# amansanghvi/Thesis

Measured on AMD Instinct MI355X. Metric: particle-updates/sec (particles x scans/s) @1081 beams, higher is better.
Workload: dtype int8 map cells (lattice log-odds), f64 poses/weights; 1 GPU; BASELINE configs[2]: room16 synthetic, 4096 particles/GPU, 1081 beams, 0.05 m grid, K=30 samples, both matcher stages, resample every step; particles_per_gpu=4096, beams=1081, parallelism=particles sharded x1

## Files before the change

thesis_amd/csrc/kernels_match.hip:

```cpp
#include <limits.h>
#include <string.h>

#include <hip/hip_ext.h>

#include "rbpf_internal.h"
#include "rbpf_device.h"

namespace rbpf {

#ifdef RBPF_STAMPS
#define MSTAMP(k) do { if (tid == 0) { long long t_ = clock64(); st_acc[k] += t_ - st_prev; st_prev = t_; } } while (0)
#else
#define MSTAMP(k) do { } while (0)
#endif

static const int MBLOCK = 512;
static const int M_COARSE = 4;
static const int M_FINE_T = 4;
static const int M_FINE_R = 4;

struct MatchArgs {
    int mode;
    int single;
    const double* ref_xy; int n_ref;
// ... 7 lines not shown
    double max_range;
    const float* sel_x; const float* sel_y; int n_sel;
    int n_coarse_rot;
    int cap_sel;
    int sc_cap;
    int p0;
    double cell_off;
    int ndt;
    int ndt_nc;
    int ndt_max_iter;
    const int32_t* dup_of;
    uint32_t* ndt_occ;
    double* ndt_aux;
};

struct __attribute__((packed, aligned(4))) MaskPair { uint32_t lo, hi; };
struct __attribute__((packed, aligned(4))) MaskTriple { uint32_t w0, w1, w2; };

struct MatchLds {
    uint32_t* occ;
    uint32_t* dil;
    uint32_t* crs;
    float* fx4; float* fy4;
    float* cx8; float* cy8;
    int* sc;
};

__host__ __device__ inline int match_crs_words(int N) { return ((N / M_COARSE) + 15) / 16; }
static const int CRS_PAD = 7;
__host__ __device__ inline int match_crs_stride(int N) { return N / M_COARSE + 2 * CRS_PAD; }
// ... 18 lines not shown
    if (nsc > (size_t)n_coarse && (size_t)n_coarse >= fine) nsc = (size_t)n_coarse;
    return base + nsc * 4;
}
int match_sc_capacity(int N, int B, size_t lds) { return (int)((lds - match_lds_base(N, B)) / 4); }

template <int N>
__device__ __forceinline__ double dpp_row_shl_f64(double x) {
    const unsigned long long b = __builtin_bit_cast(unsigned long long, x);
    const int lo = __builtin_amdgcn_update_dpp(0, (int)(uint32_t)b, 0x100 + N, 0xF, 0xF, true);
    const int hi = __builtin_amdgcn_update_dpp(0, (int)(uint32_t)(b >> 32), 0x100 + N, 0xF, 0xF, true);
    return __builtin_bit_cast(double, ((unsigned long long)(uint32_t)hi << 32) | (uint32_t)lo);
}
__device__ __forceinline__ double wave_sum_lane0_f64(double x) {
    x += __shfl_down(x, 32, 64); x += __shfl_down(x, 16, 64);
    x += dpp_row_shl_f64<8>(x); x += dpp_row_shl_f64<4>(x); x += dpp_row_shl_f64<2>(x); x += dpp_row_shl_f64<1>(x);
    return x;
}

__device__ __forceinline__ int field_hit(const MatchLds& s, int N, int u, int w) {
    if ((unsigned)u >= (unsigned)N || (unsigned)w >= (unsigned)N) return 0;
    int idx = u * (N >> 5) + (w >> 5);
    uint32_t m = 1u << (w & 31);
    return ((s.occ[idx] & m) ? 1 : 0) + ((s.dil[idx] & m) ? 1 : 0);
}
__device__ inline void match_frame_from(const MatchArgs& a, const double* pose5, double* g, double* rng, int* org) {
    double gx, gy, gth, rx, ry;
    if (a.single) {
        gx = a.guess[0]; gy = a.guess[1]; gth = a.guess[2]; rx = a.range[0]; ry = a.range[1];
    } else {
        gx = pose5[0]; gy = pose5[1]; gth = pose5[2];
// ... 23 lines not shown
    if (dup != p) { if (tid == 0) atomicAdd(&v.stats[ST_MATCH_SHARED], 1ull); return; }
    MatchLds s;
    s.occ = reinterpret_cast<uint32_t*>(smem);
    s.dil = s.occ + (size_t)N * W;
    s.crs = s.dil + (size_t)N * W;
    const int cap4 = ((a.cap_sel + 3) / 4 + 7) & ~3, cap8 = ((a.cap_sel + 7) / 8 + 7) & ~3;
    s.fx4 = reinterpret_cast<float*>(s.crs + match_crs_total(N)); s.fy4 = s.fx4 + cap4;
    s.cx8 = s.fy4 + cap4; s.cy8 = s.cx8 + cap8;
    s.sc = reinterpret_cast<int*>(s.cy8 + cap8);
    __shared__ double s_g[3], s_rng[2];
    __shared__ int s_org[2], s_nb, s_best;
    __shared__ unsigned long long s_bestc;
    __shared__ unsigned s_def[32], s_slowg;
    __shared__ double s_mom[10], s_wmom[MBLOCK / 64][10];
    __shared__ int s_tab[49];

#ifdef RBPF_STAMPS
    long long st_acc[8] = {0, 0, 0, 0, 0, 0, 0, 0}, st_prev = clock64();
#endif
    if (tid == 0) {
        match_frame_from(a, pre, s_g, s_rng, s_org);
        s_nb = 0; s_best = INT_MIN; s_bestc = 0ull; s_slowg = 0;
        for (int i = 0; i < 10; ++i) s_mom[i] = 0.0;
    }
    if (!a.single) {
        const int32_t* tab = v.tile_tab + (size_t)pre_slot * v.L * v.L;
        for (int i = tid; i < v.L * v.L; i += MBLOCK) s_tab[i] = tab[i];
    }
    if (a.mode != 0) for (int i = tid; i < N * W; i += MBLOCK) s.occ[i] = 0;
    if (tid < 32) s_def[tid] = 0;
    __syncthreads();
    const int ox = s_org[0], oy = s_org[1];

    MSTAMP(0);
    if (a.mode == 0) {
        int16_t* colmap = reinterpret_cast<int16_t*>(s.sc);
        uint32_t* rowbase = s.dil;
        for (int i = tid; i < N * a.ds; i += MBLOCK) {
            const int gyi = oy * a.ds + i, gxi = ox * a.ds + i;
            int16_t e = -1;
            if (lut_valid_g(v, gyi)) {
                const uint32_t ey = lut_at(v, gyi);
                e = (int16_t)((lut_lat(ey) << 12) | lut_cidx(ey));
                const int dev_ = lut_cidx(ey) - (gyi - (lut_lat(ey) - v.R) * v.dim + v.dim / 2);
                if (dev_ == -1) atomicOr(&s_def[(i >> 5) & 31], 1u << (i & 31));
                else if (dev_ != 0) atomicOr(&s_slowg, 1u << ((i >> 5) & 31));
                const int g0 = gyi - (i & 31);
                if ((i & 31) && !(lut_valid_g(v, g0) && lut_lat(lut_at(v, g0)) == lut_lat(ey))) atomicOr(&s_slowg, 1u << ((i >> 5) & 31));
            } else atomicOr(&s_slowg, 1u << ((i >> 5) & 31));
            colmap[i] = e;
            uint32_t rb = 0xFFFFFFFFu;
            if (lut_valid_g(v, gxi)) { const uint32_t ex = lut_at(v, gxi); rb = ((uint32_t)lut_lat(ex) << 24) | (uint32_t)lut_cidx(ex); }
            rowbase[i] = rb;
        }
        __syncthreads();
        MSTAMP(6);
        if (a.ds == 2 && 2 * W <= 32 && !v.match_stage_slow) {
            for (int q = tid; q < N * W; q += MBLOCK) {
                const int u = q / W, wv = q % W;
                const int e0 = colmap[wv * 64], e1 = colmap[wv * 64 + 32];
                const bool fast2 = !((s_slowg >> (2 * wv)) & 3u) && e0 >= 0 && e1 >= 0 && (e0 >> 12) == (e1 >> 12);
                uint32_t bits = 0;
                if (fast2) {
                    const int lat = e0 >> 12;
                    const int c0 = (oy * 2 + wv * 64) - (lat - v.R) * v.dim + v.dim / 2;
                    const int cy = max(c0 - 1, 0), wi = cy >> 5, sft = c0 - (wi << 5);
                    const unsigned long long d64 = ((unsigned long long)s_def[2 * wv + 1] << 32) | s_def[2 * wv];
                    unsigned long long acc = 0;
                    for (int du = 0; du < 2; ++du) {
                        const uint32_t rb = rowbase[u * 2 + du];
                        if (rb == 0xFFFFFFFFu) continue;
                        const int t = s_tab[(rb >> 24) * v.L + lat];
                        if (t < 0) continue;
                        const uint32_t* row = v.occ + ((size_t)t * v.dim + (rb & 0xFFFFFFu)) * v.ow;
// ... 20 lines not shown
                        if (rb == 0xFFFFFFFFu) continue;
                        for (int b = 0; b < 64; ++b) {
                            const int e = colmap[wv * 64 + b];
                            if (e < 0) continue;
                            const int t = s_tab[(rb >> 24) * v.L + (e >> 12)];
                            if (t < 0) continue;
                            const int cyb = e & 0xFFF;
                            const uint32_t wd = v.occ[((size_t)t * v.dim + (rb & 0xFFFFFFu)) * v.ow + (cyb >> 5)];
                            if ((wd >> (cyb & 31)) & 1u) bits |= 1u << (b >> 1);
                        }
                    }
                }
                s.occ[u * W + wv] = bits;
            }
        } else {
        const int SW = 4;
        const int GT = (W + 3) / 4, NRB = N / 16;
        const unsigned slowg = (a.ds != 1 || W > 32 || v.match_stage_slow) ? 0xFFFFFFFFu : s_slowg;
        const int wave = tid >> 6, ln = tid & 63;
        for (int g = 0; g < GT; ++g) {
            const int wv = g * 4 + (ln >> 4);
            const bool wv_ok = wv < W, fastw = wv_ok && !((slowg >> wv) & 1u);
            int lat = 0, wi = 0, sft = 0; uint32_t d = 0;
            if (fastw) {
                lat = colmap[wv * 32] >> 12;
                const int c0 = (oy + wv * 32) - (lat - v.R) * v.dim + v.dim / 2;
                wi = max(c0 - 1, 0) >> 5;
                sft = c0 - (wi << 5);
                d = s_def[wv];
            }
            for (int rb0 = wave; rb0 < NRB; rb0 += SW * (MBLOCK / 64)) {
                MaskPair mp[SW];
#pragma unroll
                for (int k = 0; k < SW; ++k) {
                    const int rbk = rb0 + k * (MBLOCK / 64);
                    mp[k].lo = 0; mp[k].hi = 0;
                    if (rbk >= NRB || !fastw) continue;
                    const uint32_t rb = rowbase[rbk * 16 + (ln & 15)];
                    if (rb == 0xFFFFFFFFu) continue;
                    const int t = s_tab[(rb >> 24) * v.L + lat];
                    if (t < 0) continue;
                    mp[k] = *reinterpret_cast<const MaskPair*>(v.occ + ((size_t)t * v.dim + (rb & 0xFFFFFFu)) * v.ow + wi);
                }
#pragma unroll
                for (int k = 0; k < SW; ++k) {
                    const int rbk = rb0 + k * (MBLOCK / 64), u = rbk * 16 + (ln & 15);
                    if (rbk >= NRB || !wv_ok) continue;
                    uint32_t bits;
                    if (fastw) {
                        const unsigned long long w01 = ((unsigned long long)mp[k].hi << 32) | mp[k].lo;
                        bits = sft < 32 ? (uint32_t)(w01 >> sft) : mp[k].hi;
                        if (d) {
                            const int s1 = sft - 1;
                            const uint32_t below = s1 < 0 ? bits << 1 : (uint32_t)(w01 >> s1);
                            bits = (bits & ~d) | (below & d);
                        }
                    } else {
                        bits = 0;
                        for (int du = 0; du < a.ds; ++du) {
                            const uint32_t rb = rowbase[u * a.ds + du];
                            if (rb == 0xFFFFFFFFu) continue;
                            for (int b = 0; b < 32 * a.ds; ++b) {
                                const int e = colmap[wv * 32 * a.ds + b];
                                if (e < 0) continue;
                                const int t = s_tab[(rb >> 24) * v.L + (e >> 12)];
                                if (t < 0) continue;
                                const int cy = e & 0xFFF;
                                const uint32_t wd = v.occ[((size_t)t * v.dim + (rb & 0xFFFFFFu)) * v.ow + (cy >> 5)];
                                if ((wd >> (cy & 31)) & 1u) bits |= 1u << (b / a.ds);
                            }
                        }
                    }
                    s.occ[u * W + wv] = bits;
                }
            }
        }
        }
        __syncthreads();
    } else {
        const int RP = 4;
        for (int i0 = tid; i0 < a.n_ref; i0 += RP * MBLOCK) {
          double2 pt[RP];
#pragma unroll
          for (int k = 0; k < RP; ++k) { const int i = i0 + k * MBLOCK; pt[k] = i < a.n_ref ? reinterpret_cast<const double2*>(a.ref_xy)[i] : make_double2(0.0, 0.0); }
#pragma unroll
          for (int k = 0; k < RP; ++k) {
            if (i0 + k * MBLOCK >= a.n_ref) continue;
            double rx = pt[k].x, ry = pt[k].y;
            double dx = rx - s_g[0], dy = ry - s_g[1];
            if (!(sqrt(dx * dx + dy * dy) < a.max_range)) continue;
            int u = (int)floor(rx / a.mcs + a.cell_off) - ox, w = (int)floor(ry / a.mcs + a.cell_off) - oy;
            if ((unsigned)u < (unsigned)N && (unsigned)w < (unsigned)N) atomicOr(&s.occ[u * W + (w >> 5)], 1u << (w & 31));
          }
        }
    }
    {
        const float inv = (float)(1.0 / a.mcs);
        const float FAR = -1.0e6f;
        for (int i = tid; i < cap4; i += MBLOCK) { const int b = 4 * i; const bool ok = b < a.n_sel; s.fx4[i] = ok ? a.sel_x[b] * inv : FAR; s.fy4[i] = ok ? a.sel_y[b] * inv : FAR; }
        for (int i = tid; i < cap8; i += MBLOCK) { const int b = 8 * i; const bool ok = b < a.n_sel; s.cx8[i] = ok ? a.sel_x[b] * inv : FAR; s.cy8[i] = ok ? a.sel_y[b] * inv : FAR; }
        if (tid == 0) s_nb = a.n_sel;
    }
    __syncthreads();
    if (a.ndt_occ) {
        uint32_t* dst = a.ndt_occ + (size_t)p * N * W;
        for (int i = tid; i < N * W; i += MBLOCK) dst[i] = s.occ[i];
    }
    MSTAMP(1);
    {
        const int nchunk = max(1, MBLOCK / W), rows_per = (N + nchunk - 1) / nchunk;
        const int wv = tid % W, chunk = tid / W;
        const bool row16 = W == 16;
        auto hdil = [&](int u) -> uint32_t {
            const bool inr = u >= 0 && u < N;
            const uint32_t c = inr ? s.occ[u * W + wv] : 0u;
            uint32_t lb, rb;
            if (row16) {
                lb = (uint32_t)__builtin_amdgcn_update_dpp(0, (int)(c >> 31), 0x111, 0xF, 0xF, true);
                rb = (uint32_t)__builtin_amdgcn_update_dpp(0, (int)(c << 31), 0x101, 0xF, 0xF, true);
            } else {
                lb = (inr && wv > 0) ? s.occ[u * W + wv - 1] >> 31 : 0u;
                rb = (inr && wv + 1 < W) ? s.occ[u * W + wv + 1] << 31 : 0u;
            }
            return c | (c << 1) | (c >> 1) | lb | rb;
        };
        if (chunk < nchunk) {
            const int u0 = chunk * rows_per, u1 = min(N, u0 + rows_per);
            uint32_t up = hdil(u0 - 1), mid = hdil(u0);
            for (int u = u0; u < u1; ++u) {
                const uint32_t dn = hdil(u + 1);
                s.dil[u * W + wv] = up | mid | dn;
                up = mid; mid = dn;
            }
        }
    }
    __syncthreads();
    for (int q = tid; q < (N / M_COARSE) * match_crs_words(N); q += MBLOCK) {
        const int cu = q / match_crs_words(N), h = q % match_crs_words(N);
        uint32_t out = 0;
#pragma unroll
        for (int k = 0; k < 4; ++k) {
            const int wv = 2 * h + k;
// ... 267 lines not shown
            for (int k = 0; k < 9; ++k) o[3 + k] = NAN;
            o[12] = 0.0;
        } else {
            const double sw = s_mom[0];
            double mu[3] = {s_mom[1] / sw, s_mom[2] / sw, s_mom[3] / sw};
            double c[3][3];
            c[0][0] = s_mom[4] / sw - mu[0] * mu[0]; c[0][1] = s_mom[5] / sw - mu[0] * mu[1]; c[0][2] = s_mom[6] / sw - mu[0] * mu[2];
            c[1][1] = s_mom[7] / sw - mu[1] * mu[1]; c[1][2] = s_mom[8] / sw - mu[1] * mu[2]; c[2][2] = s_mom[9] / sw - mu[2] * mu[2];
            c[1][0] = c[0][1]; c[2][0] = c[0][2]; c[2][1] = c[1][2];
            const double fl_t = (a.mcs * a.mcs) / 16.0, fl_r = (a.d0 * a.d0) / 16.0;
            c[0][0] = fmax(c[0][0], 0.0) + fl_t; c[1][1] = fmax(c[1][1], 0.0) + fl_t; c[2][2] = fmax(c[2][2], 0.0) + fl_r;
            for (int i = 0; i < 3; ++i) for (int j = 0; j < 3; ++j) o[3 + 3 * i + j] = c[i][j];
            o[12] = 0.5 * (double)full_score;
        }
        if (a.ndt_aux) {
            double* x = a.ndt_aux + (size_t)p * 5;
            x[0] = bdx / a.mcs; x[1] = bdy / a.mcs; x[2] = bth; x[3] = (double)full_score; x[4] = ok ? 1.0 : 0.0;
        }
    }
}

struct NdtCell { double mx, my, b00, b01, b11; };
__device__ inline bool ndt_cell_stats(int n, int sx, int sy, int sxx, int sxy, int syy, NdtCell& c) {
    if (n < 3) return false;
    const double nn = (double)n, mx = (double)sx / nn, my = (double)sy / nn;
    const double ca = ((double)sxx - (double)sx * mx) / (nn - 1.0);
    const double cb = ((double)sxy - (double)sx * my) / (nn - 1.0);
    const double cc = ((double)syy - (double)sy * my) / (nn - 1.0);
    const double half_tr = 0.5 * (ca + cc), disc = sqrt(0.25 * (ca - cc) * (ca - cc) + cb * cb);
    const double l1 = half_tr + disc, l2 = half_tr - disc;
    double k = 0.0;
    if (l2 < 1e-3 * l1) { k = (1e-3 * l1 - l2) / (l1 - l2); if (!(fabs(k) <= 1.79e308)) k = 0.0; }
// ... 111 lines not shown
__global__ __launch_bounds__(NBLOCK, 4) void ndt_kernel(DevView v, MatchArgs a) {
    extern __shared__ __align__(16) unsigned char smem[];
    const int N = a.N, W = N >> 5, tid = threadIdx.x, p = a.p0 + blockIdx.x;
    uint32_t* occ = reinterpret_cast<uint32_t*>(smem);
    const float* __restrict__ bx = a.sel_x;
    const float* __restrict__ by = a.sel_y;
    const float inv = (float)(1.0 / a.mcs);
    __shared__ double s_g[3], s_rng[2], s_trial[6], s_w[NBLOCK / 64][10];
    __shared__ int s_org[2], s_go;
    __shared__ float s_lut[5][16];
    __shared__ unsigned s_ok;
#ifdef RBPF_STAMPS
    long long st_acc[8] = {0, 0, 0, 0, 0, 0, 0, 0}, st_prev = clock64();
#endif
    if (a.dup_of && a.dup_of[p] != p) return;
    const double* aux = a.ndt_aux + (size_t)p * 5;
    if (aux[4] == 0.0 || a.n_sel <= 0) return;
    if (tid == 0) { match_frame(v, a, p, s_g, s_rng, s_org); s_ok = 0; }
    const int WPD = W + 2;
    {
        const uint32_t* src = a.ndt_occ + (size_t)p * N * W;
        int u = tid / W, wv = tid % W;
        const int du = NBLOCK / W, dw = NBLOCK % W;
        const int SL = 16;
        for (int i0 = tid; i0 < N * W; i0 += SL * NBLOCK) {
            uint32_t val[SL]; int dst[SL];
#pragma unroll
            for (int k = 0; k < SL; ++k) {
                const int i = i0 + k * NBLOCK;
                val[k] = i < N * W ? src[i] : 0u;
                dst[k] = (u + 1) * WPD + wv + 1;
                u += du; wv += dw;
                if (wv >= W) { wv -= W; ++u; }
            }
#pragma unroll
            for (int k = 0; k < SL; ++k)
                if (i0 + k * NBLOCK < N * W) occ[dst[k]] = val[k];
        }
        for (int i = tid; i < WPD; i += NBLOCK) { occ[i] = 0; occ[(N + 1) * WPD + i] = 0; }
        for (int i = tid; i < N; i += NBLOCK) { occ[(i + 1) * WPD] = 0; occ[(i + 1) * WPD + W + 1] = 0; }
    }
    __syncthreads();
    if (tid < 16) {
        const int b0 = tid & 1, b1 = (tid >> 1) & 1, b2 = (tid >> 2) & 1, b3 = (tid >> 3) & 1;
        NdtCell c = {0, 0, 0, 0, 0};
        const bool okc = ndt_cell_stats(b0 + b1 + b2 + b3, b2 + b3, b1 + b3, b2 + b3, b3, b1 + b3, c);
        if (okc) atomicOr(&s_ok, 1u << tid);
        s_lut[0][tid] = okc ? (float)(0.5 + c.mx) : NDT_FAR; s_lut[1][tid] = okc ? (float)(0.5 + c.my) : NDT_FAR;
        s_lut[2][tid] = okc ? (float)c.b00 : 1.0f; s_lut[3][tid] = okc ? (float)c.b01 : 0.0f; s_lut[4][tid] = okc ? (float)c.b11 : 1.0f;
    }
    const int ox = s_org[0], oy = s_org[1], nb = a.n_sel, nc = a.ndt_nc;
    const double gth = s_g[2];
    const double X0 = s_g[0] / a.mcs - (double)ox + a.cell_off, Y0 = s_g[1] / a.mcs - (double)oy + a.cell_off;
    __shared__ double s_cur[10], s_pose[3], s_step[3], s_lam;
    __shared__ int s_evals;
// ... 210 lines not shown
```

thesis_amd/csrc/rbpf_api.hip:

```cpp
#include <math.h>
#include <stdio.h>
#include <stdlib.h>
#include <string.h>

#include <algorithm>
#include <initializer_list>
#include <limits>

#include "rbpf_host.h"
#include "rbpf_scanbatch.h"

using namespace rbpf;

static thread_local std::string g_create_err;

#define HIP_TRY(h, call)                                                                           \
    do {                                                                                           \
        hipError_t e_ = (call);                                                                    \
        if (e_ != hipSuccess) {                                                                    \
            (h)->err = std::string(#call) + ": " + hipGetErrorString(e_);                          \
            return RBPF_EDEVICE;                                                                   \
        }                                                                                          \
    } while (0)

// ... 237 lines not shown
        ALLOC(h, v.upd_pose, 3 * P);
        ALLOC(h, v.prop_prep, 24 * P);
        ALLOC(h, v.prop_samp, 256 * P);
        ALLOC(h, v.stats, ST_COUNT); ALLOC(h, v.err, 1);
        ALLOC(h, v.mu_fallback, P); HIP_TRY(h, hipMemset(v.mu_fallback, 0, P * 4));
        ALLOC(h, v.ev_queue, 2); HIP_TRY(h, hipMemset(v.ev_queue, 0, 8));
        ALLOC(h, h->d_did_early, 1);
        HIP_TRY(h, hipMemset(h->d_did_early, 0, 4));
        HIP_TRY(h, h->events.create(&h->ev_weights, hipEventDisableTiming | hipEventDisableSystemFence));
        {
            v.mu_mode = env_is("RBPF_MAP_KERNEL", "window") ? MU_WINDOW : env_is("RBPF_MAP_KERNEL", "ray") ? MU_RAY : env_is("RBPF_MAP_KERNEL", "ev") ? MU_EV : MU_DEFAULT;
            v.ev_resident = env_is("RBPF_EV_RESIDENT", "0") ? 0 : 1;
            const char* eg = getenv("RBPF_EV_GRID");
            v.ev_grid = eg ? std::max(0, atoi(eg)) : 0;
            v.match_stage_slow = env_is("RBPF_MATCH_STAGE", "slow") ? 1 : 0;
            const char* ws = getenv("RBPF_WSAFE");
            v.wsafe_override = ws ? (float)atof(ws) : -1.0f;
            v.weight_entry_f64 = env_is("RBPF_WEIGHT_ENTRY", "f64") ? 1 : 0;
            v.ndt_refine = h->cfg.ndt_refine;
            h->dedup_enabled = !env_is("RBPF_MATCH_DEDUP", "0");
            {
                int cus = 0;
                if (hipDeviceGetAttribute(&cus, hipDeviceAttributeMultiprocessorCount, c.device) != hipSuccess || cus < 1) { (void)hipGetLastError(); cus = 1; }
                h->skip_discarded = !env_is("RBPF_SKIP_DISCARDED", "0");
                h->hold_back = getenv("RBPF_SKIP_DISCARDED") ? true : (long long)P > 4LL * cus;
                const bool halves = env_is("RBPF_SCAN_HALVES", "0") ? false : getenv("RBPF_SCAN_HALVES") ? true : ((long long)P >= SCAN_HALVES_MIN_PER_CU * cus && (long long)P < SCAN_HALVES_END_PER_CU * cus);
                if (halves) {
                    int least = 0, greatest = 0;
                    HIP_TRY(h, hipDeviceGetStreamPriorityRange(&least, &greatest));
                    HIP_TRY(h, hipStreamCreateWithPriority(&h->side, hipStreamNonBlocking, greatest));
                    HIP_TRY(h, h->events.create(&h->ev_fork, hipEventDisableTiming | hipEventDisableSystemFence));
                    HIP_TRY(h, h->events.create(&h->ev_half_match, hipEventDisableSystemFence));
                    HIP_TRY(h, h->events.create(&h->ev_half_weight, hipEventDisableSystemFence));
                    h->halves_first = (int)(P - std::max<size_t>(P > 1 ? 1 : 0, 3 * P / 8));
                }
            }
        }
        ALLOC(h, v.dup_of, P); v.dups_valid = 0;
        ALLOC(h, h->d_last_xy, 2 * (size_t)c.max_beams); ALLOC(h, h->d_tmp_sel, 2 * (size_t)c.max_beams);
        if (raycast_lds_bytes(c.max_beams, v.reach) > LDS_LIMIT) return fail(h, RBPF_EINVAL, "max_beams too large for the LDS window layout");
        match_geometry(c, c.cell_size, h->mN, h->mds, h->mmcs, h->md0, h->mncr);
        h->mlds = match_lds_bytes(h->mN, c.max_beams, match_max_coarse(h->mncr, 0.7, h->mmcs), match_per_rot(0.7, h->mmcs));
        if (h->mlds > LDS_LIMIT) return fail(h, RBPF_EINVAL, "matcher region does not fit in LDS for this cell_size");
        if (c.ndt_refine && ndt_cells(h->mmcs) >= 2) {
            if (ndt_lds_bytes(h->mN, c.max_beams) > LDS_LIMIT) return fail(h, RBPF_EINVAL, "NDT stage: matcher region does not fit in LDS");
            ALLOC(h, v.ndt_occ, P * (size_t)h->mN * (h->mN / 32)); ALLOC(h, v.ndt_aux, 5 * P);
        }
        ALLOC(h, h->d_match, 13 * P); ALLOC(h, h->d_bad, P); ALLOC(h, h->d_guess_full, P * (size_t)c.n_samples * 3);
        {
            ResampleBuffers& r = h->rs;
            ALLOC(h, r.T, P); ALLOC(h, r.idx, P); ALLOC(h, r.did, 1); ALLOC(h, r.slot2, P); ALLOC(h, r.dead_list, P);
            ALLOC(h, r.jobs, 2 * P); ALLOC(h, r.n_jobs, 2); ALLOC(h, r.pending_free, (size_t)v.pool_tiles); ALLOC(h, r.n_pending, 1);
            ALLOC(h, r.px2, P); ALLOC(h, r.py2, P); ALLOC(h, r.pth2, P); ALLOC(h, r.cov2, 9 * P); ALLOC(h, r.w2, P);
            ALLOC(h, r.skip, P); ALLOC(h, r.keep, P); ALLOC(h, r.plan, 2);
            HIP_TRY(h, hipMemset(r.n_pending, 0, 4)); HIP_TRY(h, hipMemset(r.n_jobs, 0, 8)); HIP_TRY(h, hipMemset(r.did, 0, 4));
            HIP_TRY(h, hipMemset(r.skip, 0, P)); HIP_TRY(h, hipMemset(r.plan, 0, 8));
        }
        HIP_TRY(h, hipMemset(v.pool, 0, (size_t)v.pool_tiles * cells));
        HIP_TRY(h, hipMemset(v.px, 0, P * 8)); HIP_TRY(h, hipMemset(v.py, 0, P * 8)); HIP_TRY(h, hipMemset(v.pth, 0, P * 8));
        HIP_TRY(h, hipMemset(v.cov, 0, 9 * P * 8));
        HIP_TRY(h, hipMemset(v.stats, 0, ST_COUNT * 8)); HIP_TRY(h, hipMemset(v.err, 0, 4));
// ... 470 lines not shown
    int N, ds, ncr; double mcs, d0;
    match_geometry(c, 1.0 / (double)cells_per_m, N, ds, mcs, d0, ncr);
    ncr = (int)floor(fabs(pose_range3[2]) / (4 * d0));
    if (ncr * 4 * d0 >= fabs(pose_range3[2])) --ncr;
    if (ncr < 0) ncr = 0;
    size_t lds = match_lds_bytes(N, h->cfg.max_beams, match_max_coarse(ncr, std::max(pose_range3[0], pose_range3[1]), mcs),
                                 match_per_rot(std::max(pose_range3[0], pose_range3[1]), mcs));
    if (lds > LDS_LIMIT) return fail(h, RBPF_EINVAL, "matcher region does not fit in LDS for this resolution");
    std::vector<float> sel(2 * (size_t)h->cfg.max_beams, 0.f);
    for (int i = 0; i < n_curr; ++i) { sel[i] = (float)curr_xy[2 * i]; sel[h->cfg.max_beams + i] = (float)curr_xy[2 * i + 1]; }
    DevTemp d_ref, d_out, d_occ, d_aux;
    HIP_TRY(h, d_ref.reserve((size_t)n_ref * 16));
    HIP_TRY(h, d_out.reserve(13 * 8));
    if (c.ndt_refine && ndt_cells(mcs) >= 2 && ndt_lds_bytes(N, h->cfg.max_beams) <= LDS_LIMIT) {
        HIP_TRY(h, d_occ.reserve((size_t)N * (N / 32) * 4));
        HIP_TRY(h, d_aux.reserve(5 * 8));
    }
    HIP_TRY(h, hipMemcpyAsync(h->d_tmp_sel, sel.data(), sel.size() * 4, hipMemcpyHostToDevice, h->stream));
    if (n_ref) HIP_TRY(h, hipMemcpyAsync(d_ref.p, ref_xy, (size_t)n_ref * 16, hipMemcpyHostToDevice, h->stream));
    launch_match_single(h->v, d_ref.as<double>(), n_ref, guess3, pose_range3, h->d_tmp_sel, h->d_tmp_sel + h->cfg.max_beams, n_curr,
                        d_out.as<double>(), N, ds, mcs, d0, ncr, h->cfg.max_beams, lds, d_occ.as<uint32_t>(), d_aux.as<double>(), h->stream);
    double out[13];
    HIP_TRY(h, hipMemcpyAsync(out, d_out.p, sizeof(out), hipMemcpyDeviceToHost, h->stream));
    int rc = check_device_error(h);
    if (rc) return rc;
    const double PI = 3.141592653589793;
    double dth = fmod(out[2] - guess3[2] + PI, 2 * PI); if (dth < 0) dth += 2 * PI; dth -= PI;
    bool valid = fabs(out[0] - guess3[0]) < fabs(pose_range3[0]) && fabs(out[1] - guess3[1]) < fabs(pose_range3[1]) &&
                 fabs(dth) < fabs(pose_range3[2]) && !(out[3] != out[3]);
    for (int i = 0; i < 3; ++i) pose_out3[i] = out[i];
    for (int i = 0; i < 9; ++i) cov_out9[i] = valid ? out[3 + i] : std::numeric_limits<double>::quiet_NaN();
// ... 2083 lines not shown
```

thesis_amd/csrc/rbpf_internal.h:

```cpp
#pragma once
#include <hip/hip_runtime.h>
#include <stdint.h>
#include <mutex>

#include "../../include/rbpf_hip.h"
#include "rbpf_math.h"
#include "rbpf_blockrelax.h"

namespace rbpf {

static const int MAX_DEVICES = 16;
inline void ensure_dynamic_lds(const void* fn, size_t bytes, size_t* set) {
    static std::mutex mu;
    std::lock_guard<std::mutex> lock(mu);
    int dev = 0;
    (void)hipGetDevice(&dev);
    const bool tracked = dev >= 0 && dev < MAX_DEVICES;
    if (tracked && bytes <= set[dev]) return;
    const hipError_t rc = hipFuncSetAttribute(fn, hipFuncAttributeMaxDynamicSharedMemorySize, (int)bytes);
    if (rc != hipSuccess) { (void)hipGetLastError(); return; }
    if (tracked) set[dev] = bytes;
}


// ... 41 lines not shown
    double*  prop_prep;
    double*  prop_samp;
    int32_t* mu_fallback;
    MapKernelMode mu_mode;
    const uint8_t* mu_skip;
    const int32_t* mu_keep;
    const int32_t* mu_n_keep;
    uint32_t* ev_queue;
    int ev_resident, ev_grid;
    uint32_t* ndt_occ; double* ndt_aux;
    int ndt_refine;
    int32_t* dup_of; int dups_valid;
    float wsafe_override;
    int weight_entry_f64;
    int match_stage_slow;
    unsigned long long* stats;
    int32_t* err;
};

struct ResampleBuffers {
    int32_t *T, *idx, *did;
    int32_t *slot2, *dead_list, *jobs;
    int32_t *n_jobs;
    int32_t *pending_free, *n_pending;
    double *px2, *py2, *pth2, *cov2, *w2;
    uint8_t* skip; int32_t* keep;
    int32_t* plan;
};

enum { ST_RAY_CELLS = 0, ST_CELLS_WRITTEN = 1, ST_GATHERS = 2, ST_SLOW_CELLS = 3,
// ... 266 lines not shown
void launch_resample_plan_late(const DevView& v, const ResampleBuffers& b, double u, double spread, hipStream_t s);
void launch_resample_copies(const DevView& v, const ResampleBuffers& b, hipStream_t s);
void launch_export_weights(const DevView& v, double* d_out, int n_global, const uint8_t* d_bad, hipStream_t s);
void launch_gather_meta(const DevView& v, const int32_t* d_local, int n, int32_t* d_out, hipStream_t s);
void launch_pack(const DevView& v, const void* d_jobs, int n_jobs, void* d_buf, hipStream_t s);
void launch_unpack(const DevView& v, const ResampleBuffers& b, const void* d_jobs, int n_jobs, const void* d_buf, hipStream_t s);
struct PackJobHost { int32_t particle, tile, x0, x1, ya, yb; long long off; };
struct UnpackJobHost { int32_t particle, pos, has, x0, x1, ya, yb, pad; long long off; };
void launch_propose_weight(const DevView& v, const double* d_match, const int32_t* d_match_of, const double* d_guesses, uint8_t* d_bad,
                           uint64_t seed, uint32_t stream, double* d_dbg_w, int p0, int n, hipStream_t s, hipEvent_t done = nullptr);
void launch_bad_weight(const DevView& v, const uint8_t* d_bad, hipStream_t s);
size_t match_lds_bytes(int N, int B, int n_coarse, int per_rot);
int match_sc_capacity(int N, int B, size_t lds);
int match_per_rot(double max_range_m, double mcs);
size_t ndt_lds_bytes(int N, int B);
int ndt_cells(double mcs);
void match_geometry(const rbpf_config& c, double cell_size, int& N, int& ds, double& mcs, double& d0, int& n_coarse_rot);
int match_max_coarse(int n_coarse_rot, double max_range_m, double mcs);
bool launch_match_particles(const DevView& v, int mode, const double* d_ref, int n_ref, double* d_out, int N, int ds,
                            double mcs, double d0, int ncr, double max_range, int cap_sel, size_t lds, int stage, int p0, int n,
                            hipStream_t s, hipEvent_t t0 = nullptr, hipEvent_t t1 = nullptr);
void launch_match_single(const DevView& v, const double* d_ref, int n_ref, const double* guess3, const double* range3,
                         const float* d_sel_x, const float* d_sel_y, int n_sel, double* d_out, int N, int ds, double mcs,
                         double d0, int ncr, int cap_sel, size_t lds, uint32_t* d_ndt_occ, double* d_ndt_aux, hipStream_t s);
void launch_match_inputs(const DevView& v, int particle, const double* guess3, double* d_all_curr, int* d_counts,
                         uint32_t* d_mask, int* d_row_cnt, double* d_ref, int cap_ref, double* d_curr, int win,
                         double match_max, hipStream_t s);
void launch_native_sincosf(const float* d_x, int n, float* d_s, float* d_c, hipStream_t s);
size_t raycast_lds_bytes(int B, int reach);
void launch_map_extent(const DevView& v, int particle, int32_t* d_box4, hipStream_t s);
// ... 33 lines not shown
```

Baseline: 2.411 million particle-updates/s.

## Restrict matcher occupancy build, dilation and NDT copy to occupied bounding box

```diff
diff --git a/thesis_amd/csrc/kernels_match.hip b/thesis_amd/csrc/kernels_match.hip
--- a/thesis_amd/csrc/kernels_match.hip
+++ b/thesis_amd/csrc/kernels_match.hip
@@ -45,6 +45,16 @@
     double* ndt_aux;
 };
 
+enum { EXT_U_LO = 0, EXT_U_HI = 1, EXT_W_LO = 2, EXT_W_HI = 3 };
+
+template <int BLOCK>
+__device__ __forceinline__ void lds_zero_words(uint32_t* p, int lo, int hi, int tid) {
+    const int a = min(hi, (lo + 3) & ~3), b = max(a, hi & ~3);
+    for (int q = (a >> 2) + tid; q < (b >> 2); q += BLOCK) reinterpret_cast<uint4*>(p)[q] = make_uint4(0u, 0u, 0u, 0u);
+    if (tid < a - lo) p[lo + tid] = 0u;
+    if (tid < hi - b) p[b + tid] = 0u;
+}
+
 struct __attribute__((packed, aligned(4))) MaskPair { uint32_t lo, hi; };
 struct __attribute__((packed, aligned(4))) MaskTriple { uint32_t w0, w1, w2; };
 
@@ -93,6 +103,16 @@
 __device__ __forceinline__ double wave_sum_lane0_f64(double x) {
     x += __shfl_down(x, 32, 64); x += __shfl_down(x, 16, 64);
     x += dpp_row_shl_f64<8>(x); x += dpp_row_shl_f64<4>(x); x += dpp_row_shl_f64<2>(x); x += dpp_row_shl_f64<1>(x);
+    return x;
+}
+
+__device__ __forceinline__ int wave_min63(int x) {
+    x = min(x, __builtin_amdgcn_mov_dpp(x, 0xB1, 0xF, 0xF, false));
+    x = min(x, __builtin_amdgcn_mov_dpp(x, 0x4E, 0xF, 0xF, false));
+    x = min(x, __builtin_amdgcn_mov_dpp(x, 0x141, 0xF, 0xF, false));
+    x = min(x, __builtin_amdgcn_mov_dpp(x, 0x140, 0xF, 0xF, false));
+    x = min(x, __builtin_amdgcn_update_dpp(x, x, 0x142, 0xA, 0xF, false));
+    x = min(x, __builtin_amdgcn_update_dpp(x, x, 0x143, 0xC, 0xF, false));
     return x;
 }
 
@@ -146,20 +166,34 @@
     __shared__ unsigned s_def[32], s_slowg;
     __shared__ double s_mom[10], s_wmom[MBLOCK / 64][10];
     __shared__ int s_tab[49];
+    static_assert(sizeof(s_wmom) >= 49 * 2 * sizeof(uint32_t), "the boxes share the per-wave moments' memory");
+    uint32_t (*const s_bb)[2] = reinterpret_cast<uint32_t (*)[2]>(&s_wmom[0][0]);
+    __shared__ int s_ext[4];
 
 #ifdef RBPF_STAMPS
     long long st_acc[8] = {0, 0, 0, 0, 0, 0, 0, 0}, st_prev = clock64();
 #endif
     if (tid == 0) {
         match_frame_from(a, pre, s_g, s_rng, s_org);
-        s_nb = 0; s_best = INT_MIN; s_bestc = 0ull; s_slowg = 0;
+        s_nb = a.n_sel; s_best = INT_MIN; s_bestc = 0ull; s_slowg = 0;
         for (int i = 0; i < 10; ++i) s_mom[i] = 0.0;
-    }
-    if (!a.single) {
-        const int32_t* tab = v.tile_tab + (size_t)pre_slot * v.L * v.L;
-        for (int i = tid; i < v.L * v.L; i += MBLOCK) s_tab[i] = tab[i];
-    }
-    if (a.mode != 0) for (int i = tid; i < N * W; i += MBLOCK) s.occ[i] = 0;
+        s_ext[EXT_U_LO] = v.match_box ? INT_MAX : 0; s_ext[EXT_U_HI] = v.match_box ? -1 : N - 1;
+        s_ext[EXT_W_LO] = v.match_box ? INT_MAX : 0; s_ext[EXT_W_HI] = v.match_box ? -1 : W - 1;
+    }
+    int my_tile = -1;
+    int4 my_bb = make_int4(INT_MAX, -1, INT_MAX, -1);
+    if (!a.single && tid < v.L * v.L) {
+        my_tile = v.tile_tab[(size_t)pre_slot * v.L * v.L + tid];
+        s_tab[tid] = my_tile;
+        if (a.mode == 0 && my_tile >= 0) my_bb = *reinterpret_cast<const int4*>(v.tile_bbox + 4 * (size_t)my_tile);
+    }
+    {
+        const float inv = (float)(1.0 / a.mcs);
+        const float FAR = -1.0e6f;
+        for (int i = tid; i < cap4; i += MBLOCK) { const int b = 4 * i; const bool ok = b < a.n_sel; s.fx4[i] = ok ? a.sel_x[b] * inv : FAR; s.fy4[i] = ok ? a.sel_y[b] * inv : FAR; }
+        for (int i = tid; i < cap8; i += MBLOCK) { const int b = 8 * i; const bool ok = b < a.n_sel; s.cx8[i] = ok ? a.sel_x[b] * inv : FAR; s.cy8[i] = ok ? a.sel_y[b] * inv : FAR; }
+    }
+    lds_zero_words<MBLOCK>(s.occ, 0, N * W, tid);
     if (tid < 32) s_def[tid] = 0;
     __syncthreads();
     const int ox = s_org[0], oy = s_org[1];
@@ -185,11 +219,52 @@
             if (lut_valid_g(v, gxi)) { const uint32_t ex = lut_at(v, gxi); rb = ((uint32_t)lut_lat(ex) << 24) | (uint32_t)lut_cidx(ex); }
             rowbase[i] = rb;
         }
+        if (tid < v.L * v.L) {
+            const bool full = my_tile >= 0 && my_bb.x <= my_bb.y && my_bb.z <= my_bb.w;
+            s_bb[tid][0] = full ? (uint32_t)my_bb.x | ((uint32_t)(my_bb.y + 1) << 16) : 0xFFFFu;
+            s_bb[tid][1] = full ? (uint32_t)my_bb.z | ((uint32_t)(my_bb.w + 1) << 16) : 0xFFFFu;
+        }
         __syncthreads();
+        if (v.match_box) {
+            const int n = N * a.ds, L = v.L, wave0 = tid & ~63, ln = tid & 63, dsh = __ffs(a.ds) - 1;
+            const int e0 = colmap[0], e1 = colmap[n - 1];
+            const uint32_t r0 = rowbase[0], r1 = rowbase[n - 1];
+            const int lc0 = e0 >= 0 ? e0 >> 12 : 0, lc1 = e1 >= 0 ? e1 >> 12 : L - 1;
+            const int lr0 = r0 != 0xFFFFFFFFu ? (int)(r0 >> 24) : 0, lr1 = r1 != 0xFFFFFFFFu ? (int)(r1 >> 24) : L - 1;
+            for (int base = wave0; base < n; base += MBLOCK) {
+                const int i = base + ln;
+                bool row_on = false, col_on = false;
+                if (i < n) {
+                    const uint32_t rb = rowbase[i];
+                    if (rb != 0xFFFFFFFFu) {
+                        const uint32_t sr = rb & 0xFFFFFFu;
+                        for (int lc = lc0; lc <= lc1; ++lc) { const uint32_t bx = s_bb[(rb >> 24) * L + lc][0]; row_on |= sr >= (bx & 0xFFFFu) && sr < (bx >> 16); }
+                    }
+                    const int e = colmap[i];
+                    if (e >= 0) {
+                        const uint32_t sc = (uint32_t)(e & 0xFFF);
+                        for (int lr = lr0; lr <= lr1; ++lr) { const uint32_t by = s_bb[lr * L + (e >> 12)][1]; col_on |= sc >= (by & 0xFFFFu) && sc < (by >> 16); }
+                    }
+                }
+                const unsigned long long mr = __ballot(row_on), mc = __ballot(col_on);
+                if (ln == 0 && mr) {
+                    atomicMin(&s_ext[EXT_U_LO], (base + __builtin_ctzll(mr)) >> dsh);
+                    atomicMax(&s_ext[EXT_U_HI], (base + 63 - __builtin_clzll(mr)) >> dsh);
+                }
+                if (ln == 0 && mc) {
+                    atomicMin(&s_ext[EXT_W_LO], ((base + __builtin_ctzll(mc)) >> dsh) >> 5);
+                    atomicMax(&s_ext[EXT_W_HI], ((base + 63 - __builtin_clzll(mc)) >> dsh) >> 5);
+                }
+            }
+            __syncthreads();
+        }
         MSTAMP(6);
+        const bool ext_on = s_ext[EXT_U_LO] <= s_ext[EXT_U_HI] && s_ext[EXT_W_LO] <= s_ext[EXT_W_HI];
+        const int xu_lo = ext_on ? s_ext[EXT_U_LO] : 0, xu_n = ext_on ? s_ext[EXT_U_HI] - xu_lo + 1 : 0;
+        const int xw_lo = ext_on ? s_ext[EXT_W_LO] : 0, xw_n = ext_on ? s_ext[EXT_W_HI] - xw_lo + 1 : 0;
         if (a.ds == 2 && 2 * W <= 32 && !v.match_stage_slow) {
-            for (int q = tid; q < N * W; q += MBLOCK) {
-                const int u = q / W, wv = q % W;
+            for (int q = tid; q < xu_n * xw_n; q += MBLOCK) {
+                const int u = xu_lo + q / xw_n, wv = xw_lo + q % xw_n;
                 const int e0 = colmap[wv * 64], e1 = colmap[wv * 64 + 32];
                 const bool fast2 = !((s_slowg >> (2 * wv)) & 3u) && e0 >= 0 && e1 >= 0 && (e0 >> 12) == (e1 >> 12);
                 uint32_t bits = 0;
@@ -240,71 +315,67 @@
                 s.occ[u * W + wv] = bits;
             }
         } else {
-        const int SW = 4;
-        const int GT = (W + 3) / 4, NRB = N / 16;
+        const int SW = 8;
+        const int nrb = (xu_n + 15) >> 4, n_items = nrb * ((xw_n + 3) >> 2);
         const unsigned slowg = (a.ds != 1 || W > 32 || v.match_stage_slow) ? 0xFFFFFFFFu : s_slowg;
         const int wave = tid >> 6, ln = tid & 63;
-        for (int g = 0; g < GT; ++g) {
-            const int wv = g * 4 + (ln >> 4);
-            const bool wv_ok = wv < W, fastw = wv_ok && !((slowg >> wv) & 1u);
-            int lat = 0, wi = 0, sft = 0; uint32_t d = 0;
-            if (fastw) {
-                lat = colmap[wv * 32] >> 12;
+        for (int it0 = wave; it0 < n_items; it0 += SW * (MBLOCK / 64)) {
+            MaskPair mp[SW]; int pos[SW], sft[SW];
+#pragma unroll
+            for (int k = 0; k < SW; ++k) {
+                const int it = it0 + k * (MBLOCK / 64), gi = it / nrb;
+                const int u = xu_lo + (it - gi * nrb) * 16 + (ln & 15), wv = xw_lo + gi * 4 + (ln >> 4);
+                mp[k].lo = 0; mp[k].hi = 0; sft[k] = -1;
+                pos[k] = (it < n_items && u < xu_lo + xu_n && wv < xw_lo + xw_n) ? (u << 8) | wv : -1;
+                if (pos[k] < 0 || ((slowg >> wv) & 1u)) continue;
+                const int lat = colmap[wv * 32] >> 12;
                 const int c0 = (oy + wv * 32) - (lat - v.R) * v.dim + v.dim / 2;
-                wi = max(c0 - 1, 0) >> 5;
-                sft = c0 - (wi << 5);
-                d = s_def[wv];
-            }
-            for (int rb0 = wave; rb0 < NRB; rb0 += SW * (MBLOCK / 64)) {
-                MaskPair mp[SW];
-#pragma unroll
-                for (int k = 0; k < SW; ++k) {
-                    const int rbk = rb0 + k * (MBLOCK / 64);
-                    mp[k].lo = 0; mp[k].hi = 0;
-                    if (rbk >= NRB || !fastw) continue;
-                    const uint32_t rb = rowbase[rbk * 16 + (ln & 15)];
-                    if (rb == 0xFFFFFFFFu) continue;
-                    const int t = s_tab[(rb >> 24) * v.L + lat];
-                    if (t < 0) continue;
-                    mp[k] = *reinterpret_cast<const MaskPair*>(v.occ + ((size_t)t * v.dim + (rb & 0xFFFFFFu)) * v.ow + wi);
-                }
-#pragma unroll
-                for (int k = 0; k < SW; ++k) {
-                    const int rbk = rb0 + k * (MBLOCK / 64), u = rbk * 16 + (ln & 15);
-                    if (rbk >= NRB || !wv_ok) continue;
-                    uint32_t bits;
-                    if (fastw) {
-                        const unsigned long long w01 = ((unsigned long long)mp[k].hi << 32) | mp[k].lo;
-                        bits = sft < 32 ? (uint32_t)(w01 >> sft) : mp[k].hi;
-                        if (d) {
-                            const int s1 = sft - 1;
-                            const uint32_t below = s1 < 0 ? bits << 1 : (uint32_t)(w01 >> s1);
-                            bits = (bits & ~d) | (below & d);
-                        }
-                    } else {
-                        bits = 0;
-                        for (int du = 0; du < a.ds; ++du) {
-                            const uint32_t rb = rowbase[u * a.ds + du];
-                            if (rb == 0xFFFFFFFFu) continue;
-                            for (int b = 0; b < 32 * a.ds; ++b) {
-                                const int e = colmap[wv * 32 * a.ds + b];
-                                if (e < 0) continue;
-                                const int t = s_tab[(rb >> 24) * v.L + (e >> 12)];
-                                if (t < 0) continue;
-                                const int cy = e & 0xFFF;
-                                const uint32_t wd = v.occ[((size_t)t * v.dim + (rb & 0xFFFFFFu)) * v.ow + (cy >> 5)];
-                                if ((wd >> (cy & 31)) & 1u) bits |= 1u << (b / a.ds);
-                            }
+                const int wi = max(c0 - 1, 0) >> 5;
+                sft[k] = c0 - (wi << 5);
+                const uint32_t rb = rowbase[u];
+                if (rb == 0xFFFFFFFFu) continue;
+                const int t = s_tab[(rb >> 24) * v.L + lat];
+                if (t < 0) continue;
+                mp[k] = *reinterpret_cast<const MaskPair*>(v.occ + ((size_t)t * v.dim + (rb & 0xFFFFFFu)) * v.ow + wi);
+            }
+#pragma unroll
+            for (int k = 0; k < SW; ++k) {
+                if (pos[k] < 0) continue;
+                const int u = pos[k] >> 8, wv = pos[k] & 0xFF;
+                uint32_t bits;
+                if (sft[k] >= 0) {
+                    const unsigned long long w01 = ((unsigned long long)mp[k].hi << 32) | mp[k].lo;
+                    bits = sft[k] < 32 ? (uint32_t)(w01 >> sft[k]) : mp[k].hi;
+                    const uint32_t d = s_def[wv];
+                    if (d) {
+                        const int s1 = sft[k] - 1;
+                        const uint32_t below = s1 < 0 ? bits << 1 : (uint32_t)(w01 >> s1);
+                        bits = (bits & ~d) | (below & d);
+                    }
+                } else {
+                    bits = 0;
+                    for (int du = 0; du < a.ds; ++du) {
+                        const uint32_t rb = rowbase[u * a.ds + du];
+                        if (rb == 0xFFFFFFFFu) continue;
+                        for (int b = 0; b < 32 * a.ds; ++b) {
+                            const int e = colmap[wv * 32 * a.ds + b];
+                            if (e < 0) continue;
+                            const int t = s_tab[(rb >> 24) * v.L + (e >> 12)];
+                            if (t < 0) continue;
+                            const int cy = e & 0xFFF;
+                            const uint32_t wd = v.occ[((size_t)t * v.dim + (rb & 0xFFFFFFu)) * v.ow + (cy >> 5)];
+                            if ((wd >> (cy & 31)) & 1u) bits |= 1u << (b / a.ds);
                         }
                     }
-                    s.occ[u * W + wv] = bits;
                 }
+                s.occ[u * W + wv] = bits;
             }
         }
         }
         __syncthreads();
     } else {
         const int RP = 4;
+        int ulo = INT_MAX, uhi = -1;
         for (int i0 = tid; i0 < a.n_ref; i0 += RP * MBLOCK) {
           double2 pt[RP];
 #pragma unroll
@@ -316,25 +387,33 @@
             double dx = rx - s_g[0], dy = ry - s_g[1];
             if (!(sqrt(dx * dx + dy * dy) < a.max_range)) continue;
             int u = (int)floor(rx / a.mcs + a.cell_off) - ox, w = (int)floor(ry / a.mcs + a.cell_off) - oy;
-            if ((unsigned)u < (unsigned)N && (unsigned)w < (unsigned)N) atomicOr(&s.occ[u * W + (w >> 5)], 1u << (w & 31));
+            if ((unsigned)u < (unsigned)N && (unsigned)w < (unsigned)N) {
+                atomicOr(&s.occ[u * W + (w >> 5)], 1u << (w & 31));
+                ulo = min(ulo, u); uhi = max(uhi, u);
+            }
           }
         }
-    }
-    {
-        const float inv = (float)(1.0 / a.mcs);
-        const float FAR = -1.0e6f;
-        for (int i = tid; i < cap4; i += MBLOCK) { const int b = 4 * i; const bool ok = b < a.n_sel; s.fx4[i] = ok ? a.sel_x[b] * inv : FAR; s.fy4[i] = ok ? a.sel_y[b] * inv : FAR; }
-        for (int i = tid; i < cap8; i += MBLOCK) { const int b = 8 * i; const bool ok = b < a.n_sel; s.cx8[i] = ok ? a.sel_x[b] * inv : FAR; s.cy8[i] = ok ? a.sel_y[b] * inv : FAR; }
-        if (tid == 0) s_nb = a.n_sel;
-    }
-    __syncthreads();
+        if (v.match_box) {
+            ulo = wave_min63(ulo); uhi = -wave_min63(-uhi);
+            if ((tid & 63) == 63 && uhi >= 0) {
+                atomicMin(&s_ext[EXT_U_LO], ulo); atomicMax(&s_ext[EXT_U_HI], uhi);
+                atomicMin(&s_ext[EXT_W_LO], 0); atomicMax(&s_ext[EXT_W_HI], W - 1);
+            }
+        }
+        __syncthreads();
+    }
+    const bool rows_on = s_ext[EXT_U_LO] <= s_ext[EXT_U_HI] && s_ext[EXT_W_LO] <= s_ext[EXT_W_HI];
+    const int u_lo = rows_on ? s_ext[EXT_U_LO] : 0, u_hi = rows_on ? s_ext[EXT_U_HI] : -1;
     if (a.ndt_occ) {
         uint32_t* dst = a.ndt_occ + (size_t)p * N * W;
-        for (int i = tid; i < N * W; i += MBLOCK) dst[i] = s.occ[i];
+        for (int i = u_lo * W + tid; i < (u_hi + 1) * W; i += MBLOCK) dst[i] = s.occ[i];
     }
     MSTAMP(1);
     {
-        const int nchunk = max(1, MBLOCK / W), rows_per = (N + nchunk - 1) / nchunk;
+        const int r_lo = max(0, u_lo - 1), r_hi = min(N - 1, u_hi + 1), nr = u_hi < u_lo ? 0 : r_hi - r_lo + 1;
+        if (nr == 0) lds_zero_words<MBLOCK>(s.dil, 0, N * W, tid);
+        else { lds_zero_words<MBLOCK>(s.dil, 0, r_lo * W, tid); lds_zero_words<MBLOCK>(s.dil, (r_hi + 1) * W, N * W, tid); }
+        const int nchunk = max(1, MBLOCK / W), rows_per = (nr + nchunk - 1) / nchunk;
         const int wv = tid % W, chunk = tid / W;
         const bool row16 = W == 16;
         auto hdil = [&](int u) -> uint32_t {
@@ -351,7 +430,7 @@
             return c | (c << 1) | (c >> 1) | lb | rb;
         };
         if (chunk < nchunk) {
-            const int u0 = chunk * rows_per, u1 = min(N, u0 + rows_per);
+            const int u0 = r_lo + chunk * rows_per, u1 = min(r_lo + nr, u0 + rows_per);
             uint32_t up = hdil(u0 - 1), mid = hdil(u0);
             for (int u = u0; u < u1; ++u) {
                 const uint32_t dn = hdil(u + 1);
@@ -649,8 +728,10 @@
             o[12] = 0.5 * (double)full_score;
         }
         if (a.ndt_aux) {
-            double* x = a.ndt_aux + (size_t)p * 5;
+            double* x = a.ndt_aux + (size_t)p * NDT_AUX;
             x[0] = bdx / a.mcs; x[1] = bdy / a.mcs; x[2] = bth; x[3] = (double)full_score; x[4] = ok ? 1.0 : 0.0;
+            const bool rows = s_ext[EXT_U_LO] <= s_ext[EXT_U_HI] && s_ext[EXT_W_LO] <= s_ext[EXT_W_HI];
+            x[5] = rows ? (double)s_ext[EXT_U_LO] : 0.0; x[6] = rows ? (double)s_ext[EXT_U_HI] : -1.0;
         }
     }
 }
@@ -792,31 +873,36 @@
     long long st_acc[8] = {0, 0, 0, 0, 0, 0, 0, 0}, st_prev = clock64();
 #endif
     if (a.dup_of && a.dup_of[p] != p) return;
-    const double* aux = a.ndt_aux + (size_t)p * 5;
+    const double* aux = a.ndt_aux + (size_t)p * NDT_AUX;
     if (aux[4] == 0.0 || a.n_sel <= 0) return;
     if (tid == 0) { match_frame(v, a, p, s_g, s_rng, s_org); s_ok = 0; }
     const int WPD = W + 2;
     {
-        const uint32_t* src = a.ndt_occ + (size_t)p * N * W;
-        int u = tid / W, wv = tid % W;
+        const int u_lo = min(max((int)aux[5], 0), N), u_hi = min((int)aux[6], N - 1), nw = max(0, u_hi - u_lo + 1) * W;
+        const uint32_t* src = a.ndt_occ + (size_t)p * N * W + (size_t)u_lo * W;
+        int u = u_lo + tid / W, wv = tid % W;
         const int du = NBLOCK / W, dw = NBLOCK % W;
         const int SL = 16;
-        for (int i0 = tid; i0 < N * W; i0 += SL * NBLOCK) {
+        for (int i0 = tid; i0 < nw; i0 += SL * NBLOCK) {
             uint32_t val[SL]; int dst[SL];
 #pragma unroll
             for (int k = 0; k < SL; ++k) {
                 const int i = i0 + k * NBLOCK;
-                val[k] = i < N * W ? src[i] : 0u;
+                val[k] = i < nw ? src[i] : 0u;
                 dst[k] = (u + 1) * WPD + wv + 1;
                 u += du; wv += dw;
                 if (wv >= W) { wv -= W; ++u; }
             }
 #pragma unroll
             for (int k = 0; k < SL; ++k)
-                if (i0 + k * NBLOCK < N * W) occ[dst[k]] = val[k];
-        }
-        for (int i = tid; i < WPD; i += NBLOCK) { occ[i] = 0; occ[(N + 1) * WPD + i] = 0; }
-        for (int i = tid; i < N; i += NBLOCK) { occ[(i + 1) * WPD] = 0; occ[(i + 1) * WPD + W + 1] = 0; }
+                if (i0 + k * NBLOCK < nw) occ[dst[k]] = val[k];
+        }
+        if (nw == 0) lds_zero_words<NBLOCK>(occ, 0, (N + 2) * WPD, tid);
+        else {
+            lds_zero_words<NBLOCK>(occ, 0, (u_lo + 1) * WPD + 1, tid);
+            lds_zero_words<NBLOCK>(occ, (u_hi + 1) * WPD + W + 1, (N + 2) * WPD, tid);
+            for (int i = u_lo + tid; i < u_hi; i += NBLOCK) { occ[(i + 1) * WPD + W + 1] = 0; occ[(i + 2) * WPD] = 0; }
+        }
     }
     __syncthreads();
     if (tid < 16) {
diff --git a/thesis_amd/csrc/rbpf_api.hip b/thesis_amd/csrc/rbpf_api.hip
--- a/thesis_amd/csrc/rbpf_api.hip
+++ b/thesis_amd/csrc/rbpf_api.hip
@@ -275,6 +275,7 @@
             const char* eg = getenv("RBPF_EV_GRID");
             v.ev_grid = eg ? std::max(0, atoi(eg)) : 0;
             v.match_stage_slow = env_is("RBPF_MATCH_STAGE", "slow") ? 1 : 0;
+            v.match_box = env_is("RBPF_MATCH_BOX", "0") ? 0 : 1;
             const char* ws = getenv("RBPF_WSAFE");
             v.wsafe_override = ws ? (float)atof(ws) : -1.0f;
             v.weight_entry_f64 = env_is("RBPF_WEIGHT_ENTRY", "f64") ? 1 : 0;
@@ -305,7 +306,7 @@
         if (h->mlds > LDS_LIMIT) return fail(h, RBPF_EINVAL, "matcher region does not fit in LDS for this cell_size");
         if (c.ndt_refine && ndt_cells(h->mmcs) >= 2) {
             if (ndt_lds_bytes(h->mN, c.max_beams) > LDS_LIMIT) return fail(h, RBPF_EINVAL, "NDT stage: matcher region does not fit in LDS");
-            ALLOC(h, v.ndt_occ, P * (size_t)h->mN * (h->mN / 32)); ALLOC(h, v.ndt_aux, 5 * P);
+            ALLOC(h, v.ndt_occ, P * (size_t)h->mN * (h->mN / 32)); ALLOC(h, v.ndt_aux, NDT_AUX * P);
         }
         ALLOC(h, h->d_match, 13 * P); ALLOC(h, h->d_bad, P); ALLOC(h, h->d_guess_full, P * (size_t)c.n_samples * 3);
         {
@@ -806,7 +807,7 @@
     HIP_TRY(h, d_out.reserve(13 * 8));
     if (c.ndt_refine && ndt_cells(mcs) >= 2 && ndt_lds_bytes(N, h->cfg.max_beams) <= LDS_LIMIT) {
         HIP_TRY(h, d_occ.reserve((size_t)N * (N / 32) * 4));
-        HIP_TRY(h, d_aux.reserve(5 * 8));
+        HIP_TRY(h, d_aux.reserve(NDT_AUX * 8));
     }
     HIP_TRY(h, hipMemcpyAsync(h->d_tmp_sel, sel.data(), sel.size() * 4, hipMemcpyHostToDevice, h->stream));
     if (n_ref) HIP_TRY(h, hipMemcpyAsync(d_ref.p, ref_xy, (size_t)n_ref * 16, hipMemcpyHostToDevice, h->stream));
diff --git a/thesis_amd/csrc/rbpf_internal.h b/thesis_amd/csrc/rbpf_internal.h
--- a/thesis_amd/csrc/rbpf_internal.h
+++ b/thesis_amd/csrc/rbpf_internal.h
@@ -79,6 +79,7 @@
     float wsafe_override;
     int weight_entry_f64;
     int match_stage_slow;
+    int match_box;
     unsigned long long* stats;
     int32_t* err;
 };
@@ -375,6 +376,7 @@
 int match_sc_capacity(int N, int B, size_t lds);
 int match_per_rot(double max_range_m, double mcs);
 size_t ndt_lds_bytes(int N, int B);
+static const int NDT_AUX = 7;
 int ndt_cells(double mcs);
 void match_geometry(const rbpf_config& c, double cell_size, int& N, int& ds, double& mcs, double& d0, int& n_coarse_rot);
 int match_max_coarse(int n_coarse_rot, double max_range_m, double mcs);
```

After: 2.426 million particle-updates/s, median of 6. No clear change (+0.6%).
